# AOS55/exorl

Hardware: AMD Instinct MI355X
Metric: gradient-steps/sec TD3+BC walker_walk batch=1024 (higher is better)
Workload: dtype bf16x3

## Files before the change

exorl_amd/csrc/agent.hip:

```cpp
#include <cmath>
#include <vector>

#include "kernels.h"

namespace exorl {

struct NetDesc {
    int in_dim = 0, out_dim = 0, H = 0, n_trunks = 0, n_heads = 0;
    int64_t W0 = 0, b0 = 0, g = 0, beta = 0, trunk_stride = 0;
    int64_t W1 = 0, b1 = 0, W2 = 0, b2 = 0, head_stride = 0;
    int64_t total = 0;
    std::vector<TensorDesc> tensors;
};

static int64_t pad4(int64_t n) { return round_up(n, 4); }

static NetDesc make_net(int in_dim, int out_dim, int H, int n_trunks, int n_heads) {
    NetDesc d;
    d.in_dim = in_dim; d.out_dim = out_dim; d.H = H; d.n_trunks = n_trunks; d.n_heads = n_heads;
    int64_t off = 0;
    auto add = [&](int64_t rows, int64_t cols) { const int64_t o = off; d.tensors.push_back({o, rows, cols}); off += pad4(rows * cols); return o; };
    auto add_trunk = [&](bool first) {
        const int64_t w = add(H, in_dim), b = add(H, 1), gg = add(H, 1), be = add(H, 1);
        if (first) { d.W0 = w; d.b0 = b; d.g = gg; d.beta = be; }
// ... 95 lines not shown
    return to_planes3(P + d.W1, d.H, d.H, d.H, sh.w1.hi, sh.w1.mid, sh.w1.lo, d.H, d.H, d.n_heads, d.head_stride, w1_plane_size(d.H), s);
}
struct Partials { float *Ph, *Pt, *Pw; };

static ShadowSpec shadow_spec(const NetDesc& d, const WeightImages& sh, const WeightImages* target) {
    ShadowSpec s{};
    s.n_trunks = d.n_trunks; s.n_heads = d.n_heads; s.in_dim = d.in_dim; s.H = d.H;
    for (int t = 0; t < d.n_trunks; ++t) s.w0_off[t] = d.W0 + t * d.trunk_stride;
    for (int i = 0; i < d.n_heads; ++i) s.w1_off[i] = d.W1 + i * d.head_stride;
    s.own = sh;
    if (target) s.target = *target;
    if (sh.w1.mid) s.own.w1 = s.target.w1 = Planes{};
    return s;
}

static int net_forward(const NetDesc& d, const float* P, const WeightImages& sh, const float* x, int64_t ldx, int rows,
                       const FwdBufs& f, bool save, bool tanh_out, int prec, hipStream_t s, const SampleSpec* sample = nullptr,
                       bool no_head = false) {
    const int H = d.H;
    const int64_t act = (int64_t)rows * H;
    const Route rt = route_of(prec, f.h1q, sh.w1, rows);
    const bool bf = rt == Route::Planes;
    if (bf && sh.w0 && trunk_fwd16_supported(H))
        EXORL_TRY(trunk_fwd16(x, ldx, sh.w0, P + d.b0, P + d.g, P + d.beta, save ? f.rstd : nullptr, f.h1q, save ? f.xhatq : Planes{}, rows,
                              d.in_dim, H, d.n_trunks, act, d.trunk_stride, s));
    else
        EXORL_TRY(trunk_fwd(x, ldx, sh.w0t, P + d.b0, P + d.g, P + d.beta, bf ? nullptr : f.h1, (save && !bf) ? f.xhat : nullptr,
                            save ? f.rstd : nullptr, bf ? f.h1q.hi : nullptr, (bf && save) ? f.xhatq.hi : nullptr, rows, d.in_dim, H,
                            d.n_trunks, act, d.trunk_stride, (int64_t)d.in_dim * H, s));
    if (rt == Route::Planes3) EXORL_TRY(to_planes3(f.h1, H, d.n_trunks * rows, H, f.h1q.hi, f.h1q.mid, f.h1q.lo, d.n_trunks * rows, H, 1, 0, 0, s));
    Product p[2];
    for (int i = 0; i < d.n_heads; ++i) {
        const int64_t t = (d.n_trunks == d.n_heads ? i : 0) * act;
        p[i] = Product{Operand(f.h1, t, f.h1q, t), Operand(P + d.W1, i * d.head_stride, sh.w1, i * w1_plane_size(H)), f.h2 + i * act,
                       P + d.b1 + i * d.head_stride, rows, H, H};
    }
    EXORL_TRY(products(rt, prec, 0, 0, p, d.n_heads, H, true, false, s));
    if (no_head) return 0;
    if (H % 4 == 0)
        EXORL_TRY(head_fwd4(f.h2, P + d.W2, P + d.b2, f.out, rows, H, d.out_dim, tanh_out ? 1 : 0, d.n_heads, act, d.head_stride,
                            (int64_t)rows * d.out_dim, s, sample));
    else
        EXORL_TRY(head_fwd(f.h2, P + d.W2, P + d.b2, f.out, rows, H, d.out_dim, tanh_out ? 1 : 0, d.n_heads, act, d.head_stride,
                           (int64_t)rows * d.out_dim, s));
    return 0;
}

static bool forward2_supported(const NetDesc& d, int prec, const WeightImages& sa, const FwdBufs& fa, const WeightImages& sb, const FwdBufs& fb, int rows) {
    const bool planes = route_of(prec, fa.h1q, sa.w1, rows) == Route::Planes && route_of(prec, fb.h1q, sb.w1, rows) == Route::Planes;
    return planes && sa.w0 && sb.w0 && trunk_fwd16_supported(d.H) && d.out_dim == 1 && d.n_heads == 2 && d.H % 4 == 0;
// ... 33 lines not shown
        if (slots > 0 && (int64_t)slots <= H) {
            for (int i = 0; i < d.n_heads; ++i) {
                q[i].head_w = P[0] + d.W2 + i * d.head_stride;
                q[i].head_part = f[0]->h2 + i * act;
            }
            *slots_a = slots;
        }
    }
    EXORL_TRY(gemm16_grouped(0, 0, q, nq, true, false, s));
    if (no_head) return 0;
    return head_fwd1_batch(hb, nq, rows, H, s);
}

static int net_backward(const NetDesc& d, const float* P, const WeightImages& sh, float* G, const Partials& pt, const float* x,
                        int64_t ldx, int rows, const FwdBufs& f, const DoutSpec& dout, const BwdBufs& b, float* dx, int dx_col0,
                        int dx_cols, int prec, hipStream_t s, const Fork& fk, FinalizeArgs* defer = nullptr, bool have_dz2 = false) {
    const int H = d.H;
    const int64_t act = (int64_t)rows * H;
    const bool paired = d.n_trunks == d.n_heads;
    Route rt = route_of(prec, f.h1q, sh.w1, rows);
    if (rt == Route::Planes3 && !b.dz2q) rt = Route::F32;
    const bool bf = rt == Route::Planes;
    const Planes none{};
    const Planes &dz2q = bf ? b.dz2q : none, &h1q = bf ? f.h1q : none, &xhatq = bf ? f.xhatq : none;
    if (have_dz2) {
    } else if (d.out_dim > 16) {
        EXORL_REQUIRE(d.n_heads == 1, "net_backward: wide heads are single-net only");
        EXORL_TRY(head_bwd_wide(dout, P + d.W2, f.h2, bf ? nullptr : b.dz2, dz2q, G ? pt.Ph : nullptr, rows, H, d.out_dim, act, d.head_stride,
                                G ? 1 : 0, s));
    } else {
        EXORL_TRY(head_bwd(dout, P + d.W2, f.h2, bf ? nullptr : b.dz2, dz2q, G ? pt.Ph : nullptr, rows, H, d.out_dim, d.n_heads, act,
                           d.head_stride, G ? 1 : 0, s, dout.mode == EXORL_DOUT_ACTOR_MU && dout.bc_part));
    }
    if (rt == Route::Planes3) EXORL_TRY(to_planes3(b.dz2, H, d.n_heads * rows, H, b.dz2q.hi, b.dz2q.mid, b.dz2q.lo, d.n_heads * rows, H, 1, 0, 0, s));
    auto trunk_of = [&](int i) { return (paired ? i : 0) * act; };
    auto wgrad = [&](int i, int r0, int kr) {
        const int64_t o = (int64_t)r0 * H;
        return Product{Operand(b.dz2, i * act + o, b.dz2q, i * act + o), Operand(f.h1, trunk_of(i) + o, f.h1q, trunk_of(i) + o),
                       G + d.W1 + i * d.head_stride, nullptr, H, H, kr};
// ... 16 lines not shown
        const int slab = (!bf && rows >= 8192) ? 1024 : rows;
        for (int r0 = 0; r0 < rows; r0 += slab) {
            for (int i = 0; i < d.n_heads; ++i) p[i] = wgrad(i, r0, rows - r0 < slab ? rows - r0 : slab);
            EXORL_TRY(products(rt, prec, 1, 1, p, d.n_heads, H, false, r0 > 0, fk.side(s)));
        }
    }
    for (int i = 0; i < d.n_heads; ++i) p[i] = dgrad(i);
    if (!paired) {
        for (int i = dgrads_done; i < d.n_heads; ++i) EXORL_TRY(products(rt, prec, 0, 1, p + i, 1, H, false, i > 0, s));
    } else if (dgrads_done == 0) {
        EXORL_TRY(products(rt, prec, 0, 1, p, d.n_heads, H, false, false, s));
    }
    const bool dx_fused = dx && !G;
    EXORL_TRY(ln_bwd(b.dh1, f.h1, f.xhat, h1q, xhatq, f.rstd, P + d.g, pt.Pt, rows, H, d.n_trunks, act, d.trunk_stride, G ? 1 : 0, s,
                     dx_fused ? sh.w0t + (int64_t)dx_col0 * H : nullptr, (int64_t)d.in_dim * H, dx_fused ? dx : nullptr, dx_cols,
                     (bf && trunk_fwd16_supported(H)) ? P + d.beta : nullptr));
    if (dx && !dx_fused)
        EXORL_TRY(head_fwd4(b.dh1, sh.w0t + (int64_t)dx_col0 * H, nullptr, dx, rows, H, dx_cols, 0, d.n_trunks, act,
                            (int64_t)d.in_dim * H, (int64_t)rows * dx_cols, s));
    if (G) {
        EXORL_TRY(outer_reduce(x, ldx, d.in_dim, b.dh1, pt.Pw, rows, H, d.n_trunks, act, s));
        EXORL_TRY(fk.join(s));
        FinalizeArgs fa{};
        fa.Ph = pt.Ph; fa.head_chunks = have_dz2 ? qhead_chunks(rows) : head_chunks(rows); fa.n_heads = d.n_heads; fa.head_stride = d.head_stride;
        fa.gW2 = d.W2; fa.gb1 = d.b1; fa.gb2 = d.b2;
        fa.Pt = pt.Pt; fa.trunk_chunks = trunk_chunks(rows); fa.n_trunks = d.n_trunks; fa.trunk_stride = d.trunk_stride;
        fa.Pw = pt.Pw; fa.w_chunks = outer_chunks(rows);
        fa.gW0 = d.W0; fa.gb0 = d.b0; fa.gg = d.g; fa.gbeta = d.beta;
        fa.H = H; fa.nout = d.out_dim; fa.in_dim = d.in_dim; fa.G = G;
        if (defer) *defer = fa;
        else EXORL_TRY(finalize_grads(fa, s));
// ... 237 lines not shown
    return FusedAdamArgs{f[EXORL_T_PARAM], f[EXORL_T_GRAD], f[EXORL_T_ADAM_M], f[EXORL_T_ADAM_V], target, c, d.n_heads,
                         {d.W1, d.W1 + d.head_stride}, reinterpret_cast<unsigned long long*>(bump)};
}
struct Step {
    hipStream_t s;
    float stddev;
    const float *noise_c, *noise_a;
    bool whole;
    bool capture;
    bool staged;
    Fork fk;
    bool fuse_opt;
    bool qfuse;
    bool metric_kernels;
    bool stats_in_phase2;
};
static Step make_step(const exorl_agent* a, hipStream_t s, float stddev, const float* noise_c, const float* noise_a, bool whole, bool capture,
                      bool staged, bool fork) {
    const int kind = a->cfg.kind;
    Step st{s, stddev, noise_c, noise_a, whole, capture, staged, Fork(a->fk, fork)};
    st.fuse_opt = whole && !a->comm && !fork;
    st.qfuse = whole && !fork && (!a->want_metrics || a->win_sums) && a->has_critic && a->critic.n_heads == 2 && a->critic.out_dim == 1 &&
               a->cfg.hidden_dim % 4 == 0 && (kind == EXORL_AGENT_TD3_BC || kind == EXORL_AGENT_TD3 || kind == EXORL_AGENT_DDPG);
    st.metric_kernels = a->win_sums ? !st.qfuse : a->want_metrics;
    st.stats_in_phase2 = st.qfuse && a->comm && kind == EXORL_AGENT_TD3_BC;
    return st;
}

static int opt_step(exorl_agent* a, const Step& st, int net, const NetDesc& d, const FinalizeArgs& pend, const AdamConst* c, float* target,
                    const ShadowSpec& spec, uint64_t* bump) {
    float** f = a->flat[net];
    hipStream_t s = st.s;
    if (st.fuse_opt) EXORL_TRY(finalize_adam(pend, fused_adam_args(a, net, d, c, target, bump), spec, s));
    else EXORL_TRY(adam_step_dev(f[EXORL_T_PARAM], f[EXORL_T_GRAD], f[EXORL_T_ADAM_M], f[EXORL_T_ADAM_V], d.total, c, target, &spec, s, bump));
    EXORL_TRY(refresh_w1_planes(d, f[EXORL_T_PARAM], net == EXORL_NET_ACTOR ? a->sh_actor : a->sh_critic, s));
    if (target) EXORL_TRY(refresh_w1_planes(d, target, a->sh_target, s));
    return 0;
}
static int opt_step_critic(exorl_agent* a, const Step& st) {
    return opt_step(a, st, EXORL_NET_CRITIC, a->critic, a->pend_c, &a->state->critic, a->flat[EXORL_NET_CRITIC_TARGET][EXORL_T_PARAM],
// ... 101 lines not shown
    if (cfg.kind == EXORL_AGENT_CRR) {
        const int n = cfg.num_value_samples;
        const float* Pc = a->flat[EXORL_NET_CRITIC][EXORL_T_PARAM];
        EXORL_TRY(repeat_sample(a->obs, a->fa.out + (int64_t)B * A, noise_a, cfg.seed, noise_a ? nullptr : &a->state->noise_counter, 1,
                                stddev, cfg.stddev_clip, a->xc_rep, B, O, A, n, s, &a->state->stddev));
        EXORL_TRY(net_forward(a->critic, Pc, a->sh_critic, a->xc_rep, W, B * n, a->fr, false, false, prec, s));
        EXORL_TRY(net_forward(a->critic, Pc, a->sh_critic, a->xc_cur, W, B, a->fc, false, false, prec, s));
        EXORL_TRY(crr_weights(a->fr.out, a->fc.out, a->crr_w, B, n, cfg.weight_func, s));
        return 0;
    }
    if ((cfg.kind == EXORL_AGENT_DDPG || cfg.kind == EXORL_AGENT_APS) && (a->want_metrics || a->win_sums))
        EXORL_TRY(sample_action(a->fa.out + (int64_t)B * A, noise_spec(a, noise_a, 1), stddev, cfg.stddev_clip, 1, a->xc_pi + O, W, B, A,
                                a->metrics + EXORL_M_ACTOR_LOGPROB, s, &a->state->stddev, cfg.world_size));
    const bool qf = st.qfuse;
    EXORL_TRY(net_forward(a->critic, a->flat[EXORL_NET_CRITIC][EXORL_T_PARAM], a->sh_critic, a->xc_pi, W, B, a->fc, true, false, prec, s,
                          nullptr, qf));
    if (cfg.kind == EXORL_AGENT_APS) {
        EXORL_TRY(sf_q(a->fc.out, a->obs + (O - cfg.sf_dim), O, a->sfq, B, cfg.sf_dim, 2, s));
        EXORL_TRY(actor_stats(a->sfq, a->stats, B, s));
    } else if (!qf) {
        EXORL_TRY(actor_stats(a->fc.out, a->stats, B, s));
    }
    return 0;
}

static int phase2(exorl_agent* a, const Step& st) {
    const auto& cfg = a->cfg;
    hipStream_t s = st.s;
    const float stddev = st.stddev;
    const bool qf = st.qfuse;
    const int B = cfg.batch, O = cfg.obs_dim, A = cfg.act_dim, W = O + A, H = cfg.hidden_dim, prec = cfg.precision;
    const float* Pa = a->flat[EXORL_NET_ACTOR][EXORL_T_PARAM];
    if (a->has_critic && cfg.kind != EXORL_AGENT_CRR) {
        DoutSpec dq{};
        dq.mode = EXORL_DOUT_ACTOR_Q; dq.q = a->fc.out; dq.stats = a->stats; dq.inv_bg = a->inv_bg; dq.alpha = cfg.alpha;
        if (cfg.kind == EXORL_AGENT_APS) { dq.q = a->sfq; dq.task = a->obs + (O - cfg.sf_dim); dq.task_ld = O; }
        dq.use_lambda = cfg.kind == EXORL_AGENT_TD3_BC;
        if (qf) EXORL_TRY(run_qhead(a, st, 1, 0));
        if (st.stats_in_phase2) {
            EXORL_TRY(reduce_pairs(a->abs_part, qhead_chunks(B), a->stats, s));
            EXORL_CHECK_HIP(hipEventRecord(a->ev_stats_ready, s));
            EXORL_CHECK_HIP(hipStreamWaitEvent(a->comm_stream, a->ev_stats_ready, 0));
            EXORL_TRY(comm_allreduce_sum(a->comm, a->stats, 4, a->comm_stream));
            EXORL_CHECK_HIP(hipEventRecord(a->ev_stats_done, a->comm_stream));
        }
        EXORL_TRY(net_backward(a->critic, a->flat[EXORL_NET_CRITIC][EXORL_T_PARAM], a->sh_critic, nullptr, a->pc, a->xc_pi, W, B, a->fc,
                               dq, a->bc, a->da, O, A, prec, s, st.fk, nullptr, qf));
    }
    const FwdBufs f = a->fa.rows_from(B, H, A);
    if (!a->has_critic)
        EXORL_TRY(net_forward(a->actor, Pa, a->sh_actor, a->xa + (int64_t)B * O, O, B, f, true, true, prec, s));
    if (st.metric_kernels)
        EXORL_TRY(actor_dmu(a->da, A, a->has_critic ? a->critic.n_trunks : 0, (int64_t)B * A, f.out, a->action,
                            a->has_critic ? nullptr : a->reward, a->crr_w, a->dpre, a->stats, a->metrics, B, A, a->inv_bg, cfg.alpha,
                            cfg.kind, stddev, s, &a->state->stddev));
    DoutSpec dm{};
    dm.mode = EXORL_DOUT_ACTOR_MU; dm.da = a->da; dm.da_nets = a->has_critic ? a->critic.n_trunks : 0; dm.mu = f.out; dm.a_data = a->action;
    dm.kind = cfg.kind; dm.inv_bg = a->inv_bg; dm.stddev = stddev; dm.stddev_ptr = &a->state->stddev; dm.w = a->crr_w;
    if (qf) {
        dm.lam_parts = a->abs_part; dm.lam_chunks = qhead_chunks(B); dm.use_lambda = cfg.kind == EXORL_AGENT_TD3_BC; dm.alpha = cfg.alpha;
        if (st.stats_in_phase2) {
            EXORL_CHECK_HIP(hipStreamWaitEvent(s, a->ev_stats_done, 0));
// ... 638 lines not shown
```

exorl_amd/csrc/fused.hip:

```cpp
#include "kernels.h"

namespace exorl {

constexpr int MAX_IN = 256;
constexpr float LN_EPS2 = 1e-5f;

constexpr int TF_ROWS = 8;
constexpr int TF_LDS_FLOATS = 35 * 1024;

__device__ __forceinline__ float tanh_fast(float x) {
    const float e = __expf(2.0f * x);
    return 1.0f - 2.0f * __frcp_rn(1.0f + e);
}

template <bool FAST>
__global__ __launch_bounds__(512) void trunk_fwd_kernel(const float* __restrict__ x, int64_t ldx,
                                                        const float* __restrict__ W0T, const float* __restrict__ b0,
                                                        const float* __restrict__ gain, const float* __restrict__ beta,
                                                        float* __restrict__ h, float* __restrict__ xhat,
                                                        float* __restrict__ rstd, unsigned short* __restrict__ hb,
                                                        unsigned short* __restrict__ xhb, int rows, int in_dim, int H,
                                                        int64_t astride, int64_t pstride, int64_t tstride, int TF_KC) {
    extern __shared__ __attribute__((aligned(16))) float smem[];
    float* ws = smem;
// ... 441 lines not shown
    static bool attr_set = false;
    if (!attr_set) {
        EXORL_CHECK_HIP(hipFuncSetAttribute((const void*)trunk_fwd_kernel<true>, hipFuncAttributeMaxDynamicSharedMemorySize, 160 * 1024));
        EXORL_CHECK_HIP(hipFuncSetAttribute((const void*)trunk_fwd_kernel<false>, hipFuncAttributeMaxDynamicSharedMemorySize, 160 * 1024));
        attr_set = true;
    }
    if (h_bf16) hipLaunchKernelGGL((trunk_fwd_kernel<true>), grid, dim3(512), lds, s, x, ldx, W0T, b0, gain, beta, h, xhat, rstd, h_bf16,
                                   xhat_bf16, rows, in_dim, H, astride, pstride, tstride, kc);
    else        hipLaunchKernelGGL((trunk_fwd_kernel<false>), grid, dim3(512), lds, s, x, ldx, W0T, b0, gain, beta, h, xhat, rstd, h_bf16,
                                   xhat_bf16, rows, in_dim, H, astride, pstride, tstride, kc);
    EXORL_LAUNCH_CHECK();
    return 0;
}

constexpr int TB_ROWS = 8;
static int tb_iters(int rows) { return rows >= 8192 ? 4 : 1; }
static int or_iters(int rows) { return rows >= 8192 ? 4 : 1; }
__device__ __forceinline__ float4 bf4_to_f4(ushort4 q) {
    return make_float4(__uint_as_float((unsigned)q.x << 16), __uint_as_float((unsigned)q.y << 16),
                       __uint_as_float((unsigned)q.z << 16), __uint_as_float((unsigned)q.w << 16));
}

__device__ __forceinline__ float wave_sum8(const float (&v)[8], int lane) {
    float a[4], b[2];
#pragma unroll
    for (int j = 0; j < 4; ++j) {
        const float keep = (lane & 1) ? v[2 * j + 1] : v[2 * j];
        const float send = (lane & 1) ? v[2 * j] : v[2 * j + 1];
        a[j] = keep + __shfl_xor(send, 1, 64);
    }
#pragma unroll
    for (int j = 0; j < 2; ++j) {
        const float keep = (lane & 2) ? a[2 * j + 1] : a[2 * j];
        const float send = (lane & 2) ? a[2 * j] : a[2 * j + 1];
        b[j] = keep + __shfl_xor(send, 2, 64);
    }
    float r = ((lane & 4) ? b[1] : b[0]) + __shfl_xor((lane & 4) ? b[0] : b[1], 4, 64);
    r += __shfl_xor(r, 8, 64);
    r += __shfl_xor(r, 16, 64);
    r += __shfl_xor(r, 32, 64);
    return r;
}

template <bool PARAMS, bool B16, bool LO, bool RECOMP>
__global__ __launch_bounds__(512) void ln_bwd_kernel(float* dh, const float* __restrict__ h, const float* __restrict__ xhat,
                                                     const unsigned short* __restrict__ hb, const unsigned short* __restrict__ xhb,
                                                     const float* __restrict__ rstd, const float* __restrict__ gain,
                                                     float* __restrict__ P, int rows, int H, int64_t astride,
                                                     int64_t pstride, const float* __restrict__ w0t, int64_t tstride,
                                                     float* __restrict__ dx, int dx_cols, const unsigned short* __restrict__ hl,
                                                     const unsigned short* __restrict__ xhl, int iters, const float* __restrict__ beta) {
    __shared__ __attribute__((aligned(16))) float red[PARAMS ? 3 * 8 * 1024 : 4];
    const int net = blockIdx.y;
    const int tid = threadIdx.x, lane = tid & 63, wave = tid >> 6;
    const int H4 = H >> 2;
    float4 g[4], be[4], pg[4], pb[4], pb0[4];
#pragma unroll
    for (int i = 0; i < 4; ++i) {
        const int c4 = lane + 64 * i;
        g[i] = c4 < H4 ? reinterpret_cast<const float4*>(gain + net * pstride)[c4] : make_float4(0.f, 0.f, 0.f, 0.f);
        be[i] = (RECOMP && c4 < H4) ? reinterpret_cast<const float4*>(beta + net * pstride)[c4] : make_float4(0.f, 0.f, 0.f, 0.f);
        pg[i] = pb[i] = pb0[i] = make_float4(0.f, 0.f, 0.f, 0.f);
    }
    for (int it = 0; it < iters; ++it) {
        const int row = blockIdx.x * TB_ROWS * iters + it * 8 + wave;
        if (row >= rows) continue;
        const int64_t o = net * astride + (int64_t)row * H;
        float4 d[4], xh[4];
        float s1 = 0.f, s2 = 0.f;
        float4 dvs[4], hvs[4];
        ushort4 xb[4], xl[4], hbv[4], hlv[4];
#pragma unroll
        for (int i = 0; i < 4; ++i) {
            const int cc = lane + 64 * i < H4 ? lane + 64 * i : 0;
            dvs[i] = reinterpret_cast<const float4*>(dh + o)[cc];
            if constexpr (B16) {
                xb[i] = reinterpret_cast<const ushort4*>(xhb + o)[cc];
                if constexpr (LO) xl[i] = reinterpret_cast<const ushort4*>(xhl + o)[cc];
                if constexpr (!RECOMP) {
                    hbv[i] = reinterpret_cast<const ushort4*>(hb + o)[cc];
                    if constexpr (LO) hlv[i] = reinterpret_cast<const ushort4*>(hl + o)[cc];
                }
            } else {
                hvs[i] = reinterpret_cast<const float4*>(h + o)[cc];
                xh[i] = reinterpret_cast<const float4*>(xhat + o)[cc];
            }
        }
#pragma unroll
        for (int i = 0; i < 4; ++i) {
            const int c4 = lane + 64 * i;
            d[i] = make_float4(0.f, 0.f, 0.f, 0.f);
            if (c4 >= H4) { xh[i] = make_float4(0.f, 0.f, 0.f, 0.f); }
            if (c4 < H4) {
                float4 hv;
                if constexpr (B16) {
                    xh[i] = bf4_to_f4(xb[i]);
                    if constexpr (LO) {
                        const float4 l2 = bf4_to_f4(xl[i]);
                        xh[i].x += l2.x; xh[i].y += l2.y; xh[i].z += l2.z; xh[i].w += l2.w;
                    }
                    if constexpr (RECOMP) {
// ... 11 lines not shown
                }
                const float4 dv = dvs[i];
                float4 dy;
                dy.x = dv.x * (1.0f - hv.x * hv.x); dy.y = dv.y * (1.0f - hv.y * hv.y);
                dy.z = dv.z * (1.0f - hv.z * hv.z); dy.w = dv.w * (1.0f - hv.w * hv.w);
                if constexpr (PARAMS) {
                    pg[i].x += dy.x * xh[i].x; pg[i].y += dy.y * xh[i].y; pg[i].z += dy.z * xh[i].z; pg[i].w += dy.w * xh[i].w;
                    pb[i].x += dy.x; pb[i].y += dy.y; pb[i].z += dy.z; pb[i].w += dy.w;
                }
                d[i].x = dy.x * g[i].x; d[i].y = dy.y * g[i].y; d[i].z = dy.z * g[i].z; d[i].w = dy.w * g[i].w;
                s1 += (d[i].x + d[i].y) + (d[i].z + d[i].w);
                s2 += (d[i].x * xh[i].x + d[i].y * xh[i].y) + (d[i].z * xh[i].z + d[i].w * xh[i].w);
            }
        }
        const float m1 = wave_sum(s1) / (float)H, m2 = wave_sum(s2) / (float)H;
        const float rs = rstd[net * (int64_t)rows + row];
        float4 dzv[4];
#pragma unroll
        for (int i = 0; i < 4; ++i) {
            const int c4 = lane + 64 * i;
            dzv[i] = make_float4(0.f, 0.f, 0.f, 0.f);
            if (c4 < H4) {
                float4 v;
                v.x = rs * (d[i].x - m1 - xh[i].x * m2); v.y = rs * (d[i].y - m1 - xh[i].y * m2);
                v.z = rs * (d[i].z - m1 - xh[i].z * m2); v.w = rs * (d[i].w - m1 - xh[i].w * m2);
                if (PARAMS || !dx) reinterpret_cast<float4*>(dh + o)[c4] = v;
                dzv[i] = v;
                if constexpr (PARAMS) { pb0[i].x += v.x; pb0[i].y += v.y; pb0[i].z += v.z; pb0[i].w += v.w; }
            }
        }
        if constexpr (!PARAMS) {
            if (dx) {
                for (int j0 = 0; j0 < dx_cols; j0 += 8) {
                    float part[8];
#pragma unroll
                    for (int j = 0; j < 8; ++j) part[j] = 0.f;
#pragma unroll
                    for (int i = 0; i < 4; ++i) {
                        const int cc = lane + 64 * i < H4 ? lane + 64 * i : 0;
                        float4 wv[8];
#pragma unroll
                        for (int j = 0; j < 8; ++j)
                            wv[j] = reinterpret_cast<const float4*>(w0t + net * tstride + (int64_t)(j0 + j < dx_cols ? j0 + j : 0) * H)[cc];
#pragma unroll
                        for (int j = 0; j < 8; ++j) part[j] += dzv[i].x * wv[j].x + dzv[i].y * wv[j].y + dzv[i].z * wv[j].z + dzv[i].w * wv[j].w;
                    }
                    const float tot = wave_sum8(part, lane);
                    const int j = j0 + (lane & 7);
                    if (lane < 8 && j < dx_cols) dx[((int64_t)net * rows + row) * dx_cols + j] = tot;
                }
            }
        }
    }
    if constexpr (PARAMS) {
        float* Pn = P + ((int64_t)net * gridDim.x + blockIdx.x) * 3 * H;
#pragma unroll
        for (int i = 0; i < 4; ++i) {
            const int c4 = lane + 64 * i;
            if (c4 < H4) {
                reinterpret_cast<float4*>(red + wave * 1024)[c4] = pg[i];
                reinterpret_cast<float4*>(red + (8 + wave) * 1024)[c4] = pb[i];
                reinterpret_cast<float4*>(red + (16 + wave) * 1024)[c4] = pb0[i];
            }
        }
        __syncthreads();
        for (int c = tid; c < H; c += 512) {
#pragma unroll
            for (int q = 0; q < 3; ++q) {
                float sacc = 0.f;
#pragma unroll
                for (int w = 0; w < 8; ++w) sacc += red[(q * 8 + w) * 1024 + c];
                Pn[q * H + c] = sacc;
            }
        }
    }
}

int ln_bwd(float* dh, const float* h, const float* xhat, const Planes& hq, const Planes& xhatq, const float* rstd, const float* gain, float* P,
           int rows, int H, int nets, int64_t astride, int64_t pstride, int want_params, hipStream_t s, const float* w0t, int64_t tstride,
           float* dx, int dx_cols, const float* beta) {
    const unsigned short *h_bf16 = hq.hi, *xhat_bf16 = xhatq.hi, *h_lo = hq.lo, *xhat_lo = xhatq.lo;
    EXORL_REQUIRE(H >= 4 && H <= 1024 && H % 4 == 0, "ln_bwd: unsupported H=%d", H);
    EXORL_REQUIRE(!dx || (!want_params && w0t && dx_cols >= 1), "ln_bwd: the dx epilogue belongs to the dgrad-only pass");
    const dim3 grid(trunk_chunks(rows), nets);
    const bool b16 = h_bf16 && xhat_bf16;
    const int iters = tb_iters(rows);
    EXORL_REQUIRE((h_lo != nullptr) == (xhat_lo != nullptr) && (!h_lo || b16), "ln_bwd: lo planes come in pairs, with the bf16 hi planes");
    const bool lo = h_lo != nullptr, rc = b16 && beta != nullptr;
#define EXORL_LNB(PA, BB, LL, RR) hipLaunchKernelGGL((ln_bwd_kernel<PA, BB, LL, RR>), grid, dim3(512), 0, s, dh, h, xhat, h_bf16, xhat_bf16, rstd, gain, P, rows, H, astride, pstride, w0t, tstride, dx, dx_cols, h_lo, xhat_lo, iters, beta)
#define EXORL_LNB2(PA) do { if (!b16) EXORL_LNB(PA, false, false, false); \
                             else if (lo && rc) EXORL_LNB(PA, true, true, true); else if (lo) EXORL_LNB(PA, true, true, false); \
                             else if (rc) EXORL_LNB(PA, true, false, true); else EXORL_LNB(PA, true, false, false); } while (0)
    if (want_params) EXORL_LNB2(true); else EXORL_LNB2(false);
#undef EXORL_LNB2
#undef EXORL_LNB
    EXORL_LAUNCH_CHECK();
    return 0;
}
int trunk_chunks(int rows) { return cdiv(rows, TB_ROWS * tb_iters(rows)); }

constexpr int OR_ROWS = 32;
__global__ __launch_bounds__(256) void outer_reduce_kernel(const float* __restrict__ u, int64_t ldu, int J,
                                                           const float* __restrict__ v, float* __restrict__ P, int rows,
                                                           int H, int64_t vstride, int iters) {
    __shared__ __attribute__((aligned(16))) float us[OR_ROWS][32];
    const int net = blockIdx.z;
    const int c = blockIdx.x * 256 + threadIdx.x;
    float* Pn = P + ((int64_t)net * gridDim.y + blockIdx.y) * (int64_t)J * H;
// ... 379 lines not shown
    }
}

int head_bwd_wide(const DoutSpec& dspec, const float* W, const float* a, float* dz, const Planes& dzq, float* P, int rows, int H,
                  int nout, int64_t astride, int64_t pstride, int want_params, hipStream_t s) {
    unsigned short *dz_bf16 = dzq.hi, *dz_lo = dzq.lo;
    EXORL_REQUIRE(nout > 16 && nout <= 32, "head_bwd_wide: nout=%d out of range", nout);
    hipLaunchKernelGGL(head_bwd_wide_kernel, dim3(cdiv(H, 256), cdiv(rows, HB_ROWS), 1), dim3(256), 0, s, dspec, W, a, dz, dz_bf16, P, rows,
                       H, nout, astride, pstride, want_params, dz_lo);
    EXORL_LAUNCH_CHECK();
    return 0;
}

int head_chunks(int rows) { return cdiv(rows, HB_ROWS); }

constexpr int QH_ROWS = 4;
template <int MODE, bool TP, bool MET = false>
__global__ __launch_bounds__(256) void qhead_kernel(const QHeadArgs g) {
    __shared__ float part[4][4 * QH_ROWS];
    __shared__ float dq[2 * QH_ROWS];
    __shared__ float met[6 * QH_ROWS];
    const int row0 = blockIdx.x * QH_ROWS;
    const int c4 = threadIdx.x, H = g.H, H4 = H >> 2;
    const int lane = threadIdx.x & 63, wave = threadIdx.x >> 6;
    const int nr = g.rows - row0 < QH_ROWS ? g.rows - row0 : QH_ROWS;
    constexpr int nn = (MODE == 0 && !TP) ? 4 : 2;
    const bool on = c4 < H4;
    float4 avs[2][QH_ROWS];
    float4 w[2];
    float dots[4 * QH_ROWS];
    float4 wvs[nn], ts[nn][QH_ROWS];
// ... 305 lines not shown
```

exorl_amd/csrc/gemm.hip:

```cpp
#include <algorithm>
#include <type_traits>
#include <vector>

#include "kernels.h"

namespace exorl {
static int g_tune_variant = 0;
static int g_prec_override = 0;
int tune_variant() { return g_tune_variant; }
int prec_override_mask() { return g_prec_override; }
}
extern "C" int exorl_gemm_tune(int32_t variant) {
    exorl::g_tune_variant = variant < 0 ? 0 : variant;
    return 0;
}
extern "C" int exorl_debug_precision_override(int32_t mask) {
    exorl::g_prec_override = mask;
    return 0;
}

namespace exorl {

struct GemmProfile {
    bool on = false;
// ... 856 lines not shown
    if (nst == NSTG) {
        group(T{}, T{});
    } else {
        group(T{}, F{});
        for (int t = NSTG; t + NSTG < nst; t += NSTG) group(F{}, F{});
        group(F{}, T{});
    }

    const bool relu = gb.relu != 0;
    auto total = [&](int pair, int i) {
        if constexpr (X6) return (accy[pair][i] + accx[pair][i]) + acc[pair][i];
        else if constexpr (X3) return accx[pair][i] + acc[pair][i];
        else return acc[pair][i];
    };
    if (P.head_part) {
#pragma unroll
        for (int ta = 0; ta < SA; ++ta) {
            float dot = 0.f;
#pragma unroll
            for (int tb = 0; tb < SB; ++tb) {
                const int nb = n0 + wn * WC + tb * 32 + 4 * h;
#pragma unroll
                for (int g4 = 0; g4 < 4; ++g4) {
                    const float4 bias = P.bias ? *reinterpret_cast<const float4*>(P.bias + nb + 8 * g4) : make_float4(0.f, 0.f, 0.f, 0.f);
                    const float4 w = *reinterpret_cast<const float4*>(P.head_w + nb + 8 * g4);
                    float4 v;
                    v.x = total(ta * SB + tb, 4 * g4 + 0) + bias.x;
                    v.y = total(ta * SB + tb, 4 * g4 + 1) + bias.y;
                    v.z = total(ta * SB + tb, 4 * g4 + 2) + bias.z;
                    v.w = total(ta * SB + tb, 4 * g4 + 3) + bias.w;
                    if (relu) { v.x = fmaxf(v.x, 0.f); v.y = fmaxf(v.y, 0.f); v.z = fmaxf(v.z, 0.f); v.w = fmaxf(v.w, 0.f); }
                    dot += (v.x * w.x + v.y * w.y) + (v.z * w.z + v.w * w.w);
                }
            }
            dot += __shfl_xor(dot, 32);
            if (h == 0) P.head_part[(int64_t)(m0 + wm * WR + ta * 32 + (lane & 31)) * (P.N / WC) + (n0 / WC + wn)] = dot;
        }
    } else {
#pragma unroll
    for (int ta = 0; ta < SA; ++ta)
#pragma unroll
        for (int tb = 0; tb < SB; ++tb) {
            const int nb = n0 + wn * WC + tb * 32 + 4 * h;
            float* crow = P.C + (int64_t)(m0 + wm * WR + ta * 32 + (lane & 31)) * P.ldc + nb;
#pragma unroll
            for (int g4 = 0; g4 < 4; ++g4) {
                if (P.n_store && nb + 8 * g4 >= P.n_store) continue;
// ... 223 lines not shown
                      "(hidden_dim and batch must be multiples of 8 in bf16 precision)", i, p.M, p.N, p.K, (long long)p.lda, (long long)p.ldb);
    }
    Gemm16Batch gb;
    memset(&gb, 0, sizeof(gb));
    const Facts16 f = gather16(probs, count, gb);
    const Pick16 pk = pick16(f);
    gb.relu = relu ? 1 : 0;
    gb.accumulate = accumulate ? 1 : 0;
    for (int i = 0; i < count; ++i)
        if (probs[i].head_part)
            EXORL_REQUIRE(probs[i].head_w && a_layout == 0 && b_layout == 0 && !accumulate && gemm16_head_slots(probs, count) > 0,
                          "gemm16_grouped: a folded head needs a forward launch on the 128 x TN kernels (ask gemm16_head_slots first)");
    EXORL_REQUIRE(!f.has_mid || pk.family == Family::p, "gemm16_grouped: three-plane operands need M %% 128 = 0, N %% 64 = 0, K %% 128 = 0 (K >= 128), 16-byte aligned "
                  "hi/mid/lo planes with pitches that are multiples of 8, 16-byte aligned C and bias, ldc %% 4 = 0 (problem 0: M=%d N=%d K=%d)",
                  probs[0].M, probs[0].N, probs[0].K);
    for (int i = 0; i < count; ++i)
        EXORL_REQUIRE(!f.has_mid || !probs[i].head_part, "gemm16_grouped: no folded head on three-plane operands");
    EXORL_REQUIRE(pk.family != Family::none, "gemm16_grouped: split-bf16 operands need M, N, K multiples of 64 and 16-byte aligned hi/lo planes");
    if (a_layout == 0 && b_layout == 0) return launch16<Form::row_row>(gb, count, f, pk, s);
    if (a_layout == 0 && b_layout == 1) return launch16<Form::row_k>(gb, count, f, pk, s);
    if (a_layout == 1 && b_layout == 1) return launch16<Form::k_k>(gb, count, f, pk, s);
    set_error("gemm16_grouped: unsupported layout combination %d %d", a_layout, b_layout);
    return 2;
}

int gemm16_grouped_mixed(const int* a_layouts, const Gemm16Problem* probs, int count, hipStream_t s) {
    EXORL_REQUIRE(count >= 1 && count <= 4, "gemm16_grouped_mixed: count %d out of range", count);
    Gemm16Batch gb;
    memset(&gb, 0, sizeof(gb));
    const Facts16 f = gather16(probs, count, gb);
    EXORL_REQUIRE(!f.has_mid, "gemm16_grouped_mixed: three-plane operands have no mixed wgrad + dgrad form");
    const Pick16 pk = pick16(f);
// ... 401 lines not shown
```

exorl_amd/csrc/kernels.h:

```cpp
#pragma once
#include <vector>

#include "numerics.h"

namespace exorl {

struct TensorDesc { int64_t off, rows, cols; };

struct SimpleCarver {
    float* base; int64_t off = 0;
    explicit SimpleCarver(float* b) : base(b) {}
    float* take(int64_t n) { float* p = base ? base + off : nullptr; off += round_up(n, 64); return p; }
};

struct Planes {
    unsigned short *hi = nullptr, *mid = nullptr, *lo = nullptr;
    __host__ __device__ Planes at(int64_t off) const { return Planes{hi ? hi + off : nullptr, mid ? mid + off : nullptr, lo ? lo + off : nullptr}; }
    __host__ __device__ explicit operator bool() const { return hi != nullptr; }
};

struct GemmProblem {
    const float* A;
    const float* B;
    float* C;
// ... 5 lines not shown
                 bool accumulate, hipStream_t s);
void gemm_planes_capture(bool allow, size_t* probe);
int gemm_planes_reserve(size_t bytes);

struct Gemm16Problem {
    const unsigned short* A;
    const unsigned short* B;
    float* C;
    const float* bias;
    int M, N, K;
    int64_t lda, ldb, ldc;
    const unsigned short* A_lo = nullptr;
    const unsigned short* B_lo = nullptr;
    const float* head_w = nullptr;
    float* head_part = nullptr;
    int n_store = 0;
    const unsigned short* A_mid = nullptr;
    const unsigned short* B_mid = nullptr;
};
int to_planes3(const float* src, int64_t ld, int rows, int cols, unsigned short* hi, unsigned short* mid, unsigned short* lo, int rows_p, int cols_p,
               int nb, int64_t src_stride, int64_t dst_stride, hipStream_t s);
int gemm16_head_slots(const Gemm16Problem* probs, int count);
int gemm16_grouped(int a_layout, int b_layout, const Gemm16Problem* probs, int count, bool relu, bool accumulate, hipStream_t s);
int gemm16_grouped_mixed(const int* a_layouts, const Gemm16Problem* probs, int count, hipStream_t s);

int ln_tanh_fwd(const float* z, const float* gain, const float* beta, float* h, float* xhat, float* rstd,
                int rows, int H, int nets, int64_t astride, int64_t pstride, hipStream_t s);
int ln_tanh_bwd(const float* dh, const float* h, const float* xhat, const float* rstd, const float* gain, float* dz,
                int rows, int H, int nets, int64_t astride, int64_t pstride, hipStream_t s);
int ln_param_grad(const float* dh, const float* h, const float* xhat, float* dgain, float* dbeta,
// ... 8 lines not shown
int trunk_fwd(const float* x, int64_t ldx, const float* W0T, const float* b0, const float* gain, const float* beta,
              float* h, float* xhat, float* rstd, unsigned short* h_bf16, unsigned short* xhat_bf16, int rows, int in_dim,
              int H, int nets, int64_t astride, int64_t pstride, int64_t tstride, hipStream_t s);
struct TrunkItem { const float* x; const unsigned short* W0b; const float *b0, *gain, *beta; float* rstd; unsigned short *hb, *xhb;
                   const unsigned short* W0l; unsigned short *hl, *xhl; };
struct TrunkBatch { TrunkItem it[4]; };
int trunk_fwd16_batch(const TrunkBatch& tb, int count, int64_t ldx, int rows, int in_dim, int H, hipStream_t s);
struct HeadItem { const float* a; const float* W; const float* b; float* out; };
struct HeadBatch { HeadItem it[4]; };
int head_fwd1_batch(const HeadBatch& hb, int count, int rows, int H, hipStream_t s);
bool trunk_fwd16_supported(int H);
int trunk_fwd16(const float* x, int64_t ldx, const Planes& W0q, const float* b0, const float* gain, const float* beta, float* rstd,
                const Planes& hq, const Planes& xhatq, int rows, int in_dim, int H, int nets, int64_t astride, int64_t pstride, hipStream_t s);
int ln_bwd(float* dh, const float* h, const float* xhat, const Planes& hq, const Planes& xhatq, const float* rstd, const float* gain, float* P,
           int rows, int H, int nets, int64_t astride, int64_t pstride, int want_params, hipStream_t s, const float* w0t, int64_t tstride,
           float* dx, int dx_cols, const float* beta);
int trunk_chunks(int rows);
int64_t knn_scratch_floats(int n_src, int n_tgt);
int knn_topk(const float* src, int n_src, const float* tgt, int n_tgt, int dim, int k, float* out, float* d2, hipStream_t s);
int outer_reduce(const float* u, int64_t ldu, int J, const float* v, float* P, int rows, int H, int nets, int64_t vstride,
                 hipStream_t s);
int outer_chunks(int rows);
struct SampleSpec {
    const float* stddev_ptr;
    const float *noise_c, *noise_a;
    uint64_t seed;
    const uint64_t* counter_ptr;
    float stddev, clip;
    float *dst_next, *dst_pi;
    int64_t dst_ld;
    int B;
// ... 335 lines not shown
```

Measured before the change: 3312.

## Fold critic Q-head gradient into GEMM epilogue and route min-Q scaling into LN backward

In the actor's pass through the twin critics, the relu-masked head-weight gradient (dz2) is now written as bf16 planes directly from the folded-head GEMM epilogue. The separate qhead kernel is skipped. The LayerNorm backward kernel gains a routed variant that sums the per-slot head partials, picks the min-Q critic, scales the dx output by the resulting weight, and writes the abs/sum partials used for the BC lambda statistics. This removes a head kernel launch and an extra pass over activations, at the cost of more epilogue work, extra stores in the GEMM, and a more specialised LN kernel.

```diff
diff --git a/exorl_amd/csrc/agent.hip b/exorl_amd/csrc/agent.hip
--- a/exorl_amd/csrc/agent.hip
+++ b/exorl_amd/csrc/agent.hip
@@ -133,9 +133,28 @@
     return s;
 }
 
+static void head_products(const NetDesc& d, const float* P, const WeightImages& sh, const FwdBufs& f, int rows, Product* p) {
+    const int H = d.H;
+    const int64_t act = (int64_t)rows * H;
+    for (int i = 0; i < d.n_heads; ++i) {
+        const int64_t t = (d.n_trunks == d.n_heads ? i : 0) * act;
+        p[i] = Product{Operand(f.h1, t, f.h1q, t), Operand(P + d.W1, i * d.head_stride, sh.w1, i * w1_plane_size(H)), f.h2 + i * act,
+                       P + d.b1 + i * d.head_stride, rows, H, H};
+    }
+}
+static int fold_slots(const NetDesc& d, const float* P, const WeightImages& sh, const FwdBufs& f, int rows, int prec) {
+    if (route_of(prec, f.h1q, sh.w1, rows) != Route::Planes || d.out_dim != 1 || d.n_heads > 2) return 0;
+    Product p[2];
+    head_products(d, P, sh, f, rows, p);
+    Gemm16Problem q[2];
+    for (int i = 0; i < d.n_heads; ++i) q[i] = g16(p[i], d.H);
+    const int slots = gemm16_head_slots(q, d.n_heads);
+    return slots <= 64 && slots <= d.H ? slots : 0;
+}
+
 static int net_forward(const NetDesc& d, const float* P, const WeightImages& sh, const float* x, int64_t ldx, int rows,
                        const FwdBufs& f, bool save, bool tanh_out, int prec, hipStream_t s, const SampleSpec* sample = nullptr,
-                       bool no_head = false) {
+                       bool no_head = false, const Planes* fold = nullptr) {
     const int H = d.H;
     const int64_t act = (int64_t)rows * H;
     const Route rt = route_of(prec, f.h1q, sh.w1, rows);
@@ -149,10 +168,18 @@
                             d.n_trunks, act, d.trunk_stride, (int64_t)d.in_dim * H, s));
     if (rt == Route::Planes3) EXORL_TRY(to_planes3(f.h1, H, d.n_trunks * rows, H, f.h1q.hi, f.h1q.mid, f.h1q.lo, d.n_trunks * rows, H, 1, 0, 0, s));
     Product p[2];
-    for (int i = 0; i < d.n_heads; ++i) {
-        const int64_t t = (d.n_trunks == d.n_heads ? i : 0) * act;
-        p[i] = Product{Operand(f.h1, t, f.h1q, t), Operand(P + d.W1, i * d.head_stride, sh.w1, i * w1_plane_size(H)), f.h2 + i * act,
-                       P + d.b1 + i * d.head_stride, rows, H, H};
+    head_products(d, P, sh, f, rows, p);
+    if (no_head && fold) {
+        EXORL_REQUIRE(rt == Route::Planes && d.n_heads <= 2, "net_forward: folded heads need the bf16 plane route");
+        Gemm16Problem q[2];
+        for (int i = 0; i < d.n_heads; ++i) {
+            q[i] = g16(p[i], H);
+            q[i].head_w = P + d.W2 + i * d.head_stride;
+            q[i].head_part = f.h2 + i * act;
+            q[i].head_dz_hi = fold->hi + i * act;
+            q[i].head_dz_lo = fold->lo ? fold->lo + i * act : nullptr;
+        }
+        return gemm16_grouped(0, 0, q, d.n_heads, true, false, s);
     }
     EXORL_TRY(products(rt, prec, 0, 0, p, d.n_heads, H, true, false, s));
     if (no_head) return 0;
@@ -216,7 +243,8 @@
 
 static int net_backward(const NetDesc& d, const float* P, const WeightImages& sh, float* G, const Partials& pt, const float* x,
                         int64_t ldx, int rows, const FwdBufs& f, const DoutSpec& dout, const BwdBufs& b, float* dx, int dx_col0,
-                        int dx_cols, int prec, hipStream_t s, const Fork& fk, FinalizeArgs* defer = nullptr, bool have_dz2 = false) {
+                        int dx_cols, int prec, hipStream_t s, const Fork& fk, FinalizeArgs* defer = nullptr, bool have_dz2 = false,
+                        const LnRoute* route = nullptr) {
     const int H = d.H;
     const int64_t act = (int64_t)rows * H;
     const bool paired = d.n_trunks == d.n_heads;
@@ -225,6 +253,7 @@
     const bool bf = rt == Route::Planes;
     const Planes none{};
     const Planes &dz2q = bf ? b.dz2q : none, &h1q = bf ? f.h1q : none, &xhatq = bf ? f.xhatq : none;
+    EXORL_REQUIRE(!route || (have_dz2 && dx && !G && bf), "net_backward: a deferred row gradient belongs to the dgrad-only pass on the bf16 route");
     if (have_dz2) {
     } else if (d.out_dim > 16) {
         EXORL_REQUIRE(d.n_heads == 1, "net_backward: wide heads are single-net only");
@@ -271,7 +300,7 @@
     const bool dx_fused = dx && !G;
     EXORL_TRY(ln_bwd(b.dh1, f.h1, f.xhat, h1q, xhatq, f.rstd, P + d.g, pt.Pt, rows, H, d.n_trunks, act, d.trunk_stride, G ? 1 : 0, s,
                      dx_fused ? sh.w0t + (int64_t)dx_col0 * H : nullptr, (int64_t)d.in_dim * H, dx_fused ? dx : nullptr, dx_cols,
-                     (bf && trunk_fwd16_supported(H)) ? P + d.beta : nullptr));
+                     (bf && trunk_fwd16_supported(H)) ? P + d.beta : nullptr, route));
     if (dx && !dx_fused)
         EXORL_TRY(head_fwd4(b.dh1, sh.w0t + (int64_t)dx_col0 * H, nullptr, dx, rows, H, dx_cols, 0, d.n_trunks, act,
                             (int64_t)d.in_dim * H, (int64_t)rows * dx_cols, s));
@@ -539,6 +568,7 @@
     bool qfuse;
     bool metric_kernels;
     bool stats_in_phase2;
+    int pi_slots;
 };
 static Step make_step(const exorl_agent* a, hipStream_t s, float stddev, const float* noise_c, const float* noise_a, bool whole, bool capture,
                       bool staged, bool fork) {
@@ -549,6 +579,9 @@
                a->cfg.hidden_dim % 4 == 0 && (kind == EXORL_AGENT_TD3_BC || kind == EXORL_AGENT_TD3 || kind == EXORL_AGENT_DDPG);
     st.metric_kernels = a->win_sums ? !st.qfuse : a->want_metrics;
     st.stats_in_phase2 = st.qfuse && a->comm && kind == EXORL_AGENT_TD3_BC;
+    st.pi_slots = 0;
+    if (st.qfuse && !a->comm && !a->win_sums && a->critic.n_trunks == 2 && a->bc.dz2q.hi)
+        st.pi_slots = fold_slots(a->critic, a->flat[EXORL_NET_CRITIC][EXORL_T_PARAM], a->sh_critic, a->fc, a->cfg.batch, a->cfg.precision);
     return st;
 }
 
@@ -680,7 +713,7 @@
                                 a->metrics + EXORL_M_ACTOR_LOGPROB, s, &a->state->stddev, cfg.world_size));
     const bool qf = st.qfuse;
     EXORL_TRY(net_forward(a->critic, a->flat[EXORL_NET_CRITIC][EXORL_T_PARAM], a->sh_critic, a->xc_pi, W, B, a->fc, true, false, prec, s,
-                          nullptr, qf));
+                          nullptr, qf, st.pi_slots > 0 ? &a->bc.dz2q : nullptr));
     if (cfg.kind == EXORL_AGENT_APS) {
         EXORL_TRY(sf_q(a->fc.out, a->obs + (O - cfg.sf_dim), O, a->sfq, B, cfg.sf_dim, 2, s));
         EXORL_TRY(actor_stats(a->sfq, a->stats, B, s));
@@ -702,7 +735,15 @@
         dq.mode = EXORL_DOUT_ACTOR_Q; dq.q = a->fc.out; dq.stats = a->stats; dq.inv_bg = a->inv_bg; dq.alpha = cfg.alpha;
         if (cfg.kind == EXORL_AGENT_APS) { dq.q = a->sfq; dq.task = a->obs + (O - cfg.sf_dim); dq.task_ld = O; }
         dq.use_lambda = cfg.kind == EXORL_AGENT_TD3_BC;
-        if (qf) EXORL_TRY(run_qhead(a, st, 1, 0));
+        LnRoute route{};
+        if (st.pi_slots > 0) {
+            const NetDesc& d = a->critic;
+            const float* Pc = a->flat[EXORL_NET_CRITIC][EXORL_T_PARAM];
+            for (int i = 0; i < 2; ++i) { route.part[i] = a->fc.h2 + i * (int64_t)B * H; route.b2[i] = Pc + d.b2 + i * d.head_stride; }
+            route.slots = st.pi_slots; route.inv_bg = a->inv_bg; route.abs_part = a->abs_part;
+        } else if (qf) {
+            EXORL_TRY(run_qhead(a, st, 1, 0));
+        }
         if (st.stats_in_phase2) {
             EXORL_TRY(reduce_pairs(a->abs_part, qhead_chunks(B), a->stats, s));
             EXORL_CHECK_HIP(hipEventRecord(a->ev_stats_ready, s));
@@ -711,7 +752,7 @@
             EXORL_CHECK_HIP(hipEventRecord(a->ev_stats_done, a->comm_stream));
         }
         EXORL_TRY(net_backward(a->critic, a->flat[EXORL_NET_CRITIC][EXORL_T_PARAM], a->sh_critic, nullptr, a->pc, a->xc_pi, W, B, a->fc,
-                               dq, a->bc, a->da, O, A, prec, s, st.fk, nullptr, qf));
+                               dq, a->bc, a->da, O, A, prec, s, st.fk, nullptr, qf, st.pi_slots > 0 ? &route : nullptr));
     }
     const FwdBufs f = a->fa.rows_from(B, H, A);
     if (!a->has_critic)
diff --git a/exorl_amd/csrc/fused.hip b/exorl_amd/csrc/fused.hip
--- a/exorl_amd/csrc/fused.hip
+++ b/exorl_amd/csrc/fused.hip
@@ -1,3 +1,5 @@
+#include <type_traits>
+
 #include "kernels.h"
 
 namespace exorl {
@@ -479,6 +481,8 @@
 }
 
 constexpr int TB_ROWS = 8;
+constexpr int QH_ROWS = 4;
+struct LnNoRoute {};
 static int tb_iters(int rows) { return rows >= 8192 ? 4 : 1; }
 static int or_iters(int rows) { return rows >= 8192 ? 4 : 1; }
 __device__ __forceinline__ float4 bf4_to_f4(ushort4 q) {
@@ -507,19 +511,24 @@
     return r;
 }
 
-template <bool PARAMS, bool B16, bool LO, bool RECOMP>
+template <bool PARAMS, bool B16, bool LO, bool RECOMP, bool ROUTE = false>
 __global__ __launch_bounds__(512) void ln_bwd_kernel(float* dh, const float* __restrict__ h, const float* __restrict__ xhat,
                                                      const unsigned short* __restrict__ hb, const unsigned short* __restrict__ xhb,
                                                      const float* __restrict__ rstd, const float* __restrict__ gain,
                                                      float* __restrict__ P, int rows, int H, int64_t astride,
                                                      int64_t pstride, const float* __restrict__ w0t, int64_t tstride,
                                                      float* __restrict__ dx, int dx_cols, const unsigned short* __restrict__ hl,
-                                                     const unsigned short* __restrict__ xhl, int iters, const float* __restrict__ beta) {
+                                                     const unsigned short* __restrict__ xhl, int iters, const float* __restrict__ beta,
+                                                     const std::conditional_t<ROUTE, LnRoute, LnNoRoute> rt) {
+    static_assert(!ROUTE || !PARAMS, "the routed epilogue belongs to the dgrad-only pass");
     __shared__ __attribute__((aligned(16))) float red[PARAMS ? 3 * 8 * 1024 : 4];
+    __shared__ float qmin[ROUTE ? 4 * TB_ROWS : 1];
     const int net = blockIdx.y;
     const int tid = threadIdx.x, lane = tid & 63, wave = tid >> 6;
     const int H4 = H >> 2;
     float4 g[4], be[4], pg[4], pb[4], pb0[4];
+    float qb[2] = {0.f, 0.f};
+    if constexpr (ROUTE) { qb[0] = rt.b2[0][0]; qb[1] = rt.b2[1][0]; }
 #pragma unroll
     for (int i = 0; i < 4; ++i) {
         const int c4 = lane + 64 * i;
@@ -535,6 +544,13 @@
         float s1 = 0.f, s2 = 0.f;
         float4 dvs[4], hvs[4];
         ushort4 xb[4], xl[4], hbv[4], hlv[4];
+        float qp[2] = {0.f, 0.f}, rs_early = 0.f;
+        if constexpr (ROUTE) {
+            rs_early = rstd[net * (int64_t)rows + row];
+            const int64_t sl = (int64_t)row * rt.slots + (lane < rt.slots ? lane : 0);
+            qp[0] = rt.part[0][sl];
+            qp[1] = rt.part[1][sl];
+        }
 #pragma unroll
         for (int i = 0; i < 4; ++i) {
             const int cc = lane + 64 * i < H4 ? lane + 64 * i : 0;
@@ -550,6 +566,23 @@
                 hvs[i] = reinterpret_cast<const float4*>(h + o)[cc];
                 xh[i] = reinterpret_cast<const float4*>(xhat + o)[cc];
             }
+        }
+        float dq = 1.0f;
+        if constexpr (ROUTE) {
+            float q1 = 0.f, q2 = 0.f;
+            if (lane >= rt.slots) qp[0] = qp[1] = 0.f;
+            for (int j0 = 0; j0 < rt.slots; j0 += 8) {
+#pragma unroll
+                for (int k = 0; k < 8; ++k) {
+                    q1 += __int_as_float(__builtin_amdgcn_readlane(__float_as_int(qp[0]), j0 + k));
+                    q2 += __int_as_float(__builtin_amdgcn_readlane(__float_as_int(qp[1]), j0 + k));
+                }
+            }
+            q1 += qb[0];
+            q2 += qb[1];
+            const float w1 = q1 < q2 ? 1.0f : (q1 == q2 ? 0.5f : 0.0f);
+            dq = -rt.inv_bg * (net == 0 ? w1 : 1.0f - w1);
+            if (net == 0 && lane == 0) qmin[it * TB_ROWS + wave] = fminf(q1, q2);
         }
 #pragma unroll
         for (int i = 0; i < 4; ++i) {
@@ -591,7 +624,7 @@
             }
         }
         const float m1 = wave_sum(s1) / (float)H, m2 = wave_sum(s2) / (float)H;
-        const float rs = rstd[net * (int64_t)rows + row];
+        const float rs = ROUTE ? rs_early : rstd[net * (int64_t)rows + row];
         float4 dzv[4];
 #pragma unroll
         for (int i = 0; i < 4; ++i) {
@@ -601,13 +634,13 @@
                 float4 v;
                 v.x = rs * (d[i].x - m1 - xh[i].x * m2); v.y = rs * (d[i].y - m1 - xh[i].y * m2);
                 v.z = rs * (d[i].z - m1 - xh[i].z * m2); v.w = rs * (d[i].w - m1 - xh[i].w * m2);
-                if (PARAMS || !dx) reinterpret_cast<float4*>(dh + o)[c4] = v;
+                if (PARAMS || (!ROUTE && !dx)) reinterpret_cast<float4*>(dh + o)[c4] = v;
                 dzv[i] = v;
                 if constexpr (PARAMS) { pb0[i].x += v.x; pb0[i].y += v.y; pb0[i].z += v.z; pb0[i].w += v.w; }
             }
         }
         if constexpr (!PARAMS) {
-            if (dx) {
+            if (ROUTE || dx) {
                 for (int j0 = 0; j0 < dx_cols; j0 += 8) {
                     float part[8];
 #pragma unroll
@@ -624,9 +657,20 @@
                     }
                     const float tot = wave_sum8(part, lane);
                     const int j = j0 + (lane & 7);
-                    if (lane < 8 && j < dx_cols) dx[((int64_t)net * rows + row) * dx_cols + j] = tot;
+                    if (lane < 8 && j < dx_cols) dx[((int64_t)net * rows + row) * dx_cols + j] = ROUTE ? dq * tot : tot;
                 }
             }
+        }
+    }
+    if constexpr (ROUTE) {
+        __syncthreads();
+        constexpr int CPI = TB_ROWS / QH_ROWS;
+        const int chunk = blockIdx.x * CPI * iters + tid, row0 = chunk * QH_ROWS;
+        if (net == 0 && tid < CPI * iters && row0 < rows) {
+            float sa = 0.f, sm = 0.f;
+            for (int r = 0; r < QH_ROWS && row0 + r < rows; ++r) { const float m = qmin[tid * QH_ROWS + r]; sa += fabsf(m); sm += m; }
+            rt.abs_part[2 * chunk] = sa;
+            rt.abs_part[2 * chunk + 1] = sm;
         }
     }
     if constexpr (PARAMS) {
@@ -655,7 +699,7 @@
 
 int ln_bwd(float* dh, const float* h, const float* xhat, const Planes& hq, const Planes& xhatq, const float* rstd, const float* gain, float* P,
            int rows, int H, int nets, int64_t astride, int64_t pstride, int want_params, hipStream_t s, const float* w0t, int64_t tstride,
-           float* dx, int dx_cols, const float* beta) {
+           float* dx, int dx_cols, const float* beta, const LnRoute* route) {
     const unsigned short *h_bf16 = hq.hi, *xhat_bf16 = xhatq.hi, *h_lo = hq.lo, *xhat_lo = xhatq.lo;
     EXORL_REQUIRE(H >= 4 && H <= 1024 && H % 4 == 0, "ln_bwd: unsupported H=%d", H);
     EXORL_REQUIRE(!dx || (!want_params && w0t && dx_cols >= 1), "ln_bwd: the dx epilogue belongs to the dgrad-only pass");
@@ -664,11 +708,17 @@
     const int iters = tb_iters(rows);
     EXORL_REQUIRE((h_lo != nullptr) == (xhat_lo != nullptr) && (!h_lo || b16), "ln_bwd: lo planes come in pairs, with the bf16 hi planes");
     const bool lo = h_lo != nullptr, rc = b16 && beta != nullptr;
-#define EXORL_LNB(PA, BB, LL, RR) hipLaunchKernelGGL((ln_bwd_kernel<PA, BB, LL, RR>), grid, dim3(512), 0, s, dh, h, xhat, h_bf16, xhat_bf16, rstd, gain, P, rows, H, astride, pstride, w0t, tstride, dx, dx_cols, h_lo, xhat_lo, iters, beta)
+#define EXORL_LNB(PA, BB, LL, RR) hipLaunchKernelGGL((ln_bwd_kernel<PA, BB, LL, RR>), grid, dim3(512), 0, s, dh, h, xhat, h_bf16, xhat_bf16, rstd, gain, P, rows, H, astride, pstride, w0t, tstride, dx, dx_cols, h_lo, xhat_lo, iters, beta, LnNoRoute{})
+#define EXORL_LNR(LL, RR) hipLaunchKernelGGL((ln_bwd_kernel<false, true, LL, RR, true>), grid, dim3(512), 0, s, dh, h, xhat, h_bf16, xhat_bf16, rstd, gain, P, rows, H, astride, pstride, w0t, tstride, dx, dx_cols, h_lo, xhat_lo, iters, beta, *route)
 #define EXORL_LNB2(PA) do { if (!b16) EXORL_LNB(PA, false, false, false); \
                              else if (lo && rc) EXORL_LNB(PA, true, true, true); else if (lo) EXORL_LNB(PA, true, true, false); \
                              else if (rc) EXORL_LNB(PA, true, false, true); else EXORL_LNB(PA, true, false, false); } while (0)
-    if (want_params) EXORL_LNB2(true); else EXORL_LNB2(false);
+    if (route) {
+        EXORL_REQUIRE(dx && b16 && nets == 2 && route->slots >= 1 && route->slots <= 64 && route->part[0] && route->part[1] && route->abs_part,
+                      "ln_bwd: the routed epilogue is the twin critics' dgrad-only pass on the bf16 images (nets=%d slots=%d)", nets, route->slots);
+        if (lo && rc) EXORL_LNR(true, true); else if (lo) EXORL_LNR(true, false); else if (rc) EXORL_LNR(false, true); else EXORL_LNR(false, false);
+    } else if (want_params) EXORL_LNB2(true); else EXORL_LNB2(false);
+#undef EXORL_LNR
 #undef EXORL_LNB2
 #undef EXORL_LNB
     EXORL_LAUNCH_CHECK();
@@ -1078,7 +1128,6 @@
 
 int head_chunks(int rows) { return cdiv(rows, HB_ROWS); }
 
-constexpr int QH_ROWS = 4;
 template <int MODE, bool TP, bool MET = false>
 __global__ __launch_bounds__(256) void qhead_kernel(const QHeadArgs g) {
     __shared__ float part[4][4 * QH_ROWS];
diff --git a/exorl_amd/csrc/gemm.hip b/exorl_amd/csrc/gemm.hip
--- a/exorl_amd/csrc/gemm.hip
+++ b/exorl_amd/csrc/gemm.hip
@@ -894,9 +894,12 @@
         else return acc[pair][i];
     };
     if (P.head_part) {
+        unsigned short* const dzh = P.head_dz_hi;
+        unsigned short* const dzl = P.head_dz_lo;
 #pragma unroll
         for (int ta = 0; ta < SA; ++ta) {
             float dot = 0.f;
+            const int64_t orow = (int64_t)(m0 + wm * WR + ta * 32 + (lane & 31)) * P.ldc;
 #pragma unroll
             for (int tb = 0; tb < SB; ++tb) {
                 const int nb = n0 + wn * WC + tb * 32 + 4 * h;
@@ -911,6 +914,11 @@
                     v.w = total(ta * SB + tb, 4 * g4 + 3) + bias.w;
                     if (relu) { v.x = fmaxf(v.x, 0.f); v.y = fmaxf(v.y, 0.f); v.z = fmaxf(v.z, 0.f); v.w = fmaxf(v.w, 0.f); }
                     dot += (v.x * w.x + v.y * w.y) + (v.z * w.z + v.w * w.w);
+                    if (dzh) {
+                        const float4 dz = make_float4(v.x > 0.f ? w.x : 0.f, v.y > 0.f ? w.y : 0.f, v.z > 0.f ? w.z : 0.f, v.w > 0.f ? w.w : 0.f);
+                        *reinterpret_cast<ushort4*>(dzh + orow + nb + 8 * g4) = bf16_bits4(dz);
+                        if (dzl) *reinterpret_cast<ushort4*>(dzl + orow + nb + 8 * g4) = bf16_lo_bits4(dz);
+                    }
                 }
             }
             dot += __shfl_xor(dot, 32);
@@ -1164,8 +1172,13 @@
     EXORL_REQUIRE(!f.has_mid || pk.family == Family::p, "gemm16_grouped: three-plane operands need M %% 128 = 0, N %% 64 = 0, K %% 128 = 0 (K >= 128), 16-byte aligned "
                   "hi/mid/lo planes with pitches that are multiples of 8, 16-byte aligned C and bias, ldc %% 4 = 0 (problem 0: M=%d N=%d K=%d)",
                   probs[0].M, probs[0].N, probs[0].K);
-    for (int i = 0; i < count; ++i)
+    for (int i = 0; i < count; ++i) {
         EXORL_REQUIRE(!f.has_mid || !probs[i].head_part, "gemm16_grouped: no folded head on three-plane operands");
+        EXORL_REQUIRE(!probs[i].head_dz_hi || (probs[i].head_part && relu && reinterpret_cast<uintptr_t>(probs[i].head_dz_hi) % 8 == 0 &&
+                                                reinterpret_cast<uintptr_t>(probs[i].head_dz_lo) % 8 == 0),
+                      "gemm16_grouped: head_dz planes belong to a folded head of a relu launch, 8-byte aligned");
+        EXORL_REQUIRE(probs[i].head_dz_hi || !probs[i].head_dz_lo, "gemm16_grouped: a head_dz lo plane without its hi plane");
+    }
     EXORL_REQUIRE(pk.family != Family::none, "gemm16_grouped: split-bf16 operands need M, N, K multiples of 64 and 16-byte aligned hi/lo planes");
     if (a_layout == 0 && b_layout == 0) return launch16<Form::row_row>(gb, count, f, pk, s);
     if (a_layout == 0 && b_layout == 1) return launch16<Form::row_k>(gb, count, f, pk, s);
diff --git a/exorl_amd/csrc/kernels.h b/exorl_amd/csrc/kernels.h
--- a/exorl_amd/csrc/kernels.h
+++ b/exorl_amd/csrc/kernels.h
@@ -43,6 +43,8 @@
     const unsigned short* B_lo = nullptr;
     const float* head_w = nullptr;
     float* head_part = nullptr;
+    unsigned short* head_dz_hi = nullptr;
+    unsigned short* head_dz_lo = nullptr;
     int n_store = 0;
     const unsigned short* A_mid = nullptr;
     const unsigned short* B_mid = nullptr;
@@ -81,7 +83,8 @@
                 const Planes& hq, const Planes& xhatq, int rows, int in_dim, int H, int nets, int64_t astride, int64_t pstride, hipStream_t s);
 int ln_bwd(float* dh, const float* h, const float* xhat, const Planes& hq, const Planes& xhatq, const float* rstd, const float* gain, float* P,
            int rows, int H, int nets, int64_t astride, int64_t pstride, int want_params, hipStream_t s, const float* w0t, int64_t tstride,
-           float* dx, int dx_cols, const float* beta);
+           float* dx, int dx_cols, const float* beta, const struct LnRoute* route = nullptr);
+struct LnRoute { const float* part[2]; const float* b2[2]; int slots; float inv_bg; float* abs_part; };
 int trunk_chunks(int rows);
 int64_t knn_scratch_floats(int n_src, int n_tgt);
 int knn_topk(const float* src, int n_src, const float* tgt, int n_tgt, int dim, int k, float* out, float* d2, hipStream_t s);
```

After: 3363 (median of 5 runs). 1.5% higher.
